# CarbonMatrixLab/AbX

Hardware: AMD Instinct MI355X
Metric: diffusion-steps/sec (100 samples, ~350-res complex) (higher is better)
Workload: dtype f32; 1 GPU; L352: L=352 (Lab 228 + antigen 124), 100 samples of one complex over 1 GPU(s), 1 step = ScoreNetwork (3 passes) + get_prev + reverse, seeded random weights, ESM off; L=352, samples_total=100, chunk=auto, parallelism=sample-shard x1, no collective in the step

## Files before the change

abx_amd/_lib.py:

```python
import ctypes as C
import os

_HERE = os.path.dirname(os.path.abspath(__file__))
LIB_PATH = os.environ.get('ABX_HIP_LIB') or os.path.join(_HERE, 'csrc', 'libabx_hip.so')

c_f = C.c_void_p
LL = C.c_longlong
I = C.c_int
F = C.c_float


class AbxGemm(C.Structure):
    _fields_ = [
        ('A', c_f), ('sAb', LL), ('sAm', LL), ('sAk', LL),
        ('B', c_f), ('sBb', LL), ('sBk', LL), ('sBn', LL),
        ('C', c_f), ('sCb', LL), ('sCm', LL),
        ('M', I), ('N', I), ('K', I), ('batch', I),
        ('c_transposed', I),
        ('ln_stats', c_f), ('sSb', LL),
        ('ln_csum', c_f),
        ('ln_eps', F),
        ('a_relu', I),
        ('bias', c_f),
        ('alpha', F),
# ... 94 lines not shown
class AbxLinearPack(C.Structure):
    _fields_ = [('Wt', c_f), ('csum', c_f), ('bias', c_f), ('planes', C.c_void_p), ('b_exp', I), ('K', I), ('N', I)]


class AbxLinearSrc(C.Structure):
    _fields_ = [('W', c_f), ('b', c_f), ('rows', I), ('glu', I)]


class AbxTriMulPack(C.Structure):
    _fields_ = [('glu', AbxLinearPack), ('out', AbxLinearPack), ('gate', AbxLinearPack)]


class AbxTriAttnPack(C.Structure):
    _fields_ = [('qkv', AbxLinearPack), ('gate', AbxLinearPack), ('pair', AbxLinearPack), ('out', AbxLinearPack)]


class AbxScoreArgs(C.Structure):
    _fields_ = [
        ('init_q', c_f), ('init_t', c_f), ('delta_q', c_f), ('cur_t', c_f), ('fixed_mask', c_f),
        ('t', c_f), ('t_is_f32', I),
        ('score_norms', c_f), ('num_sigma', I), ('num_omega', I), ('discrete_sigma', c_f), ('discrete_omega', c_f),
        ('exp_max_sigma', F), ('exp_min_sigma', F),
        ('min_b', F), ('bdiff', F),
        ('coord_scale', F),
        ('position_scale', F),
        ('rot_score', c_f), ('trans_score', c_f), ('rigids', c_f),
        ('B', I), ('L', I),
    ]


class AbxReverseArgs(C.Structure):
    _fields_ = [
        ('rigid_in', c_f), ('rigid_is_f64', I),
        ('seq_in', c_f),
        ('rot_score', c_f), ('trans_score', c_f), ('ts_is_f32', I), ('logits', c_f),
        ('diffuse_mask', c_f), ('t', c_f), ('dt', F),
        ('z_rot', c_f), ('z_trans', c_f), ('jumps', c_f),
        ('u_jumps', c_f),
        ('dt_dev', c_f),
        ('seed', C.c_ulonglong), ('sample_ids', c_f), ('step', I),
        ('step_dev', c_f),
        ('exp_max_sigma', F), ('exp_min_sigma', F), ('min_b', F), ('bdiff', F), ('coord_scale', F), ('rate_const', F),
        ('noise_scale', F), ('center', I),
        ('rigid_out', c_f), ('seq_out', c_f), ('rates_out', c_f), ('jumps_out', c_f),
        ('B', I), ('L', I),
    ]


class AbxGuidanceArgs(C.Structure):
    _fields_ = [
        ('atom14', c_f), ('atom_mask', c_f), ('aatype', c_f), ('chain_id', c_f),
        ('residx', c_f),
        ('radius', c_f), ('frame_trans', c_f),
        ('overlap_tolerance', F), ('between_chain_factor', F), ('bond_tolerance_factor', F), ('w_clash', F), ('w_bond', F), ('w_angle', F),
        ('energy', c_f), ('grad_atom', c_f), ('grad_trans', c_f), ('grad_rot', c_f),
        ('B', I), ('L', I),
    ]


_S = c_f

_PROTOS = {
    'abx_version': (I, []),
    'abx_last_error_string': (C.c_char_p, []),
    'abx_init': (I, [I]),
    'abx_gemm': (I, [C.POINTER(AbxGemm), _S]),
    'abx_gemm_side': (I, [C.POINTER(AbxGemm), C.POINTER(AbxGemm), _S]),
    'abx_gemm_check_modes': (I, [C.POINTER(AbxGemm)]),
    'abx_gemm_planes_ok': (I, [LL]),
    'abx_split_weights_f16': (I, [c_f, LL, LL, I, I, I, C.c_void_p, _S]),
    'abx_ipa_tail': (I, [C.POINTER(AbxIpaTail), _S]),
    'abx_heads_tail': (I, [C.POINTER(AbxHeadsTail), _S]),
    'abx_gemm3_occupancy': (I, [I]),
    'abx_row_stats': (I, [c_f, LL, LL, LL, I, I, I, F, c_f, _S]),
    'abx_layernorm': (I, [c_f, LL, LL, I, c_f, c_f, F, c_f, LL, c_f, LL, _S]),
    'abx_tri_attn_fwd': (I, [C.POINTER(AbxTriAttn), _S]),
    'abx_seq_attn_fwd': (I, [c_f, c_f, c_f, c_f, c_f, I, I, I, I, F, _S]),
    'abx_ipa_pack': (I, [c_f, c_f, c_f, c_f, c_f, c_f, I, I, F, _S]),
    'abx_ipa_attn': (I, [c_f, c_f, c_f, c_f, c_f, c_f, c_f, c_f, c_f, c_f, c_f, I, I, _S]),
    'abx_debug_poison_lds': (I, [C.c_uint, _S]),
    'abx_ipa_weights': (I, [c_f, c_f, c_f, c_f, c_f, c_f, c_f, c_f, c_f, c_f, I, I, _S]),
    'abx_ipa_pair': (I, [c_f, c_f, c_f, I, I, _S]),
    'abx_ipa_attn_workspace_bytes': (C.c_longlong, [I, I]),
    'abx_ipa_qpack_bytes': (C.c_longlong, [I, I]),
    'abx_timestep_embedding': (I, [c_f, c_f, I, I, c_f, _S]),
    'abx_assemble_seq': (I, [c_f, LL, c_f, c_f, I, c_f, c_f, c_f, c_f, c_f, I, I, I, I, _S]),
    'abx_assemble_pair': (I, [c_f, LL, c_f, c_f, c_f, c_f, c_f, c_f, c_f, c_f, I, I, I, I, _S]),
    'abx_opm_features': (I, [c_f, c_f, LL, c_f, I, I, I, _S]),
    'abx_opm_out_fwd': (I, [c_f, LL, c_f, c_f, c_f, I, I, c_f, I, _S]),
    'abx_assemble_pair_bias': (I, [c_f, LL, c_f, c_f, c_f, c_f, c_f, c_f, c_f, C.c_void_p, I, c_f, c_f, F, c_f, I, I, c_f, I, _S]),
    'abx_pair_mask': (I, [c_f, c_f, I, I, I, _S]),
    'abx_transpose_last2': (I, [c_f, c_f, I, I, I, I, _S]),
    'abx_pair_embed_features': (I, [c_f, c_f, c_f, c_f, c_f, c_f, c_f, c_f, c_f, c_f, c_f, c_f, I, I, _S]),
    'abx_relpos_block': (I, [c_f, c_f, c_f, I, I, I, I, I, _S]),
    'abx_gather_rows': (I, [c_f, c_f, c_f, c_f, LL, LL, I, _S]),
    'abx_frames_init': (I, [c_f, I, c_f, c_f, c_f, c_f, c_f, c_f, I, F, _S]),
    'abx_rigid_update': (I, [c_f, c_f, c_f, c_f, c_f, c_f, c_f, c_f, I, F, _S]),
    'abx_scores': (I, [C.POINTER(AbxScoreArgs), _S]),
    'abx_torsion_finalize': (I, [c_f, c_f, c_f, c_f, I, _S]),
    'abx_seq_head_atoms': (I, [c_f, c_f, c_f, c_f, c_f, c_f, c_f, c_f, c_f, c_f, c_f, c_f, I, _S]),
    'abx_prev_pos': (I, [c_f, c_f, I, c_f, I, I, _S]),
    'abx_plddt': (I, [c_f, c_f, I, I, _S]),
    'abx_igso3_tables': (I, [c_f, c_f, I, I, I, c_f, c_f, c_f, _S]),
    'abx_reverse_step': (I, [C.POINTER(AbxReverseArgs), _S]),
    'abx_clash_grad_workspace_bytes': (LL, [I, I]),
    'abx_clash_grad': (I, [C.POINTER(AbxGuidanceArgs), c_f, _S]),
    'abx_pack_linear_bytes': (LL, [I, I]),
    'abx_pack_linear': (I, [C.POINTER(AbxLinearSrc), I, I, c_f, c_f, I, c_f, C.POINTER(AbxLinearPack), _S]),
    'abx_transition_workspace_bytes': (LL, [LL, I, I]),
    'abx_transition_fwd': (I, [C.POINTER(AbxLinearPack), C.POINTER(AbxLinearPack), c_f, LL, I, c_f, c_f, I, _S]),
    'abx_tri_mul_workspace_bytes': (LL, [I, I]),
    'abx_tri_mul_workspace_init': (I, [c_f, I, I, _S]),
    'abx_tri_mul_fwd': (I, [C.POINTER(AbxTriMulPack), c_f, c_f, c_f, I, I, I, c_f, c_f, I, _S]),
    'abx_tri_attn_block_workspace_bytes': (LL, [I, I]),
    'abx_tri_attn_block_fwd': (I, [C.POINTER(AbxTriAttnPack), c_f, c_f, I, I, I, I, c_f, c_f, I, _S]),
}

EXPORTED = tuple(_PROTOS)
_lib = None


class AbxHipError(RuntimeError):
    pass


def library_path():
    return LIB_PATH


def load():
    global _lib
    if _lib is not None:
        return _lib
    if not os.path.exists(LIB_PATH):
        raise AbxHipError(f'{LIB_PATH} not found: build it with `make -C abx_amd/csrc` (no CPU fallback exists)')
    lib = C.CDLL(LIB_PATH)
    for name, (res, args) in _PROTOS.items():
        fn = getattr(lib, name)
        fn.restype = res
        fn.argtypes = args
    if lib.abx_version() != 1:
        raise AbxHipError('libabx_hip ABI version mismatch')
    _lib = lib
    return lib


def check(rc, what):
    if rc != 0:
        msg = load().abx_last_error_string()
        raise AbxHipError(f'{what} failed (rc={rc}): {msg.decode() if msg else ""}')
```

abx_amd/csrc/ipa.hip:

```cpp
#include "common.h"
#include "abx_hip.h"

namespace {

constexpr int H = 12, SQK = 16, SV = 16, PQK = 4, PV = 8, CZ = 128;
constexpr int QREC = SQK + 3 * PQK;
constexpr int VREC = SV + 3 * PV;
constexpr int NPROJ = H * SQK + H * (SQK + SV) + 3 * H * PQK + 3 * H * (PQK + PV);
constexpr int OFF_KV = H * SQK;
constexpr int OFF_QP = OFF_KV + H * (SQK + SV);
constexpr int OFF_KVP = OFF_QP + 3 * H * PQK;
constexpr int NFEAT = H * SV + 3 * H * PV + H * PV + H * CZ;

constexpr int IPA_THREADS = 512;
constexpr int IQ = 12;
constexpr int HG = 4, NHG = H / HG;

__global__ __launch_bounds__(256) void ipa_pack_kernel(const float* __restrict__ proj, const float* __restrict__ rots,
                                                       const float* __restrict__ trans, float* __restrict__ qpack,
                                                       float* __restrict__ kpack, float* __restrict__ vpack, int B, int L,
                                                       float w_s) {
    const int NIB = (L + IQ - 1) / IQ, LQ = NIB * IQ;
    const long long idx = (long long)blockIdx.x * 256 + threadIdx.x;
    if (idx >= (long long)B * LQ * H) return;
// ... 267 lines not shown
        const long long row = (long long)b * L + i0 + iq;
        const float* R = rots + row * 9;
        const float* t = trans + row * 3;
        const float* g = opt + (iq * HG + hl) * VREC + SV + pt * 3;
        float loc[3];
#pragma unroll
        for (int r = 0; r < 3; ++r) {
            const float it = -(R[0 * 3 + r] * t[0] + R[1 * 3 + r] * t[1] + R[2 * 3 + r] * t[2]);
            loc[r] = it + (R[0 * 3 + r] * g[0] + R[1 * 3 + r] * g[1] + R[2 * 3 + r] * g[2]);
        }
        float* fo = feat + row * NFEAT;
#pragma unroll
        for (int r = 0; r < 3; ++r) fo[H * SV + r * (H * PV) + n] = loc[r];
        fo[H * SV + 3 * H * PV + n] = sqrtf(loc[0] * loc[0] + loc[1] * loc[1] + loc[2] * loc[2] + 1e-8f);
    }
    ISTAMP(7)
}

constexpr int PAIR_WAVES = 4;
#ifndef ABX_PAIR_UZ
#define ABX_PAIR_UZ 8
#endif
constexpr int UZ = ABX_PAIR_UZ;

__global__ __launch_bounds__(PAIR_WAVES * 64) void ipa_pair_kernel(const float* __restrict__ attn, const float* __restrict__ z,
                                                                   float* __restrict__ feat, long long rows, int L) {
    typedef float f32x2 __attribute__((ext_vector_type(2)));
    __shared__ __attribute__((aligned(16))) float wl[PAIR_WAVES][UZ * H];
    const int lane = threadIdx.x & 63, wave = threadIdx.x >> 6;
    const long long row = (long long)blockIdx.x * PAIR_WAVES + wave;
    if (row >= rows) return;
    const float* __restrict__ wr = attn + row * L * H;
    const float* __restrict__ zr = z + row * L * CZ + lane * 2;
    float* ws = wl[wave];
    const int nw = L * HG;
    f32x2 acc[H];
#pragma unroll
    for (int h = 0; h < H; ++h) acc[h] = (f32x2){0.f, 0.f};
    f32x2 za[UZ], zb[UZ];
    float wa[NHG], wb[NHG];
    auto request = [&](int j0, f32x2 (&zd)[UZ], float (&wd)[NHG]) {
#pragma unroll
        for (int u = 0; u < UZ; ++u) zd[u] = *reinterpret_cast<const f32x2*>(zr + (long long)min(j0 + u, L - 1) * CZ);
#pragma unroll
        for (int q = 0; q < NHG; ++q) wd[q] = wr[(long long)q * nw + min(j0 * HG + (lane & (UZ * HG - 1)), nw - 1)];
    };
    auto sum_step = [&](int j0, const f32x2 (&zd)[UZ], const float (&wd)[NHG]) {
#pragma unroll
        for (int q = 0; q < NHG; ++q) ws[q * (UZ * HG) + (lane & (UZ * HG - 1))] = wd[q];
        __builtin_amdgcn_fence(__ATOMIC_RELEASE, "wavefront");
        __builtin_amdgcn_wave_barrier();
        __builtin_amdgcn_fence(__ATOMIC_ACQUIRE, "wavefront");
#pragma unroll
        for (int u = 0; u < UZ; ++u) {
            if (j0 + u < L) {
                f32x4 w4[H / 4];
#pragma unroll
                for (int q = 0; q < NHG; ++q) w4[q] = *reinterpret_cast<const f32x4*>(ws + q * (UZ * HG) + u * HG);
#pragma unroll
                for (int h = 0; h < H; ++h) {
                    const float wh = w4[h >> 2][h & 3];
                    acc[h][0] = fmaf(wh, zd[u][0], acc[h][0]);
                    acc[h][1] = fmaf(wh, zd[u][1], acc[h][1]);
                }
            }
        }
        __builtin_amdgcn_fence(__ATOMIC_RELEASE, "wavefront");
        __builtin_amdgcn_wave_barrier();
    };
    request(0, za, wa);
    for (int j0 = 0; j0 < L; j0 += 2 * UZ) {
        if (j0 + UZ < L) request(j0 + UZ, zb, wb);
        sum_step(j0, za, wa);
        if (j0 + UZ < L) {
            if (j0 + 2 * UZ < L) request(j0 + 2 * UZ, za, wa);
            sum_step(j0 + UZ, zb, wb);
        }
    }
    float* fo = feat + row * NFEAT + (H * SV + 4 * H * PV) + lane * 2;
#pragma unroll
    for (int h = 0; h < H; ++h) *reinterpret_cast<f32x2*>(fo + h * CZ) = acc[h];
}

}

extern "C" int abx_ipa_pack(const float* proj, const float* rots, const float* trans, float* qpack, float* kpack,
                            float* vpack, int B, int L, float scalar_weight, hipStream_t st) {
    ABX_REQUIRE(proj && rots && trans && qpack && kpack && vpack && B > 0 && L > 0, "abx_ipa_pack: bad args");
    const long long n = (long long)B * ((L + IQ - 1) / IQ) * IQ * H;
    hipLaunchKernelGGL(ipa_pack_kernel, dim3((unsigned)((n + 255) / 256)), dim3(256), 0, st, proj, rots, trans, qpack, kpack,
                       vpack, B, L, scalar_weight);
    return abx_check_launch("abx_ipa_pack");
}

extern "C" long long abx_ipa_qpack_bytes(int B, int L) {
    return (long long)B * ((L + IQ - 1) / IQ) * IQ * H * QREC * sizeof(float);
}

extern "C" long long abx_ipa_attn_workspace_bytes(int B, int L) {
    return (long long)B * L * L * H * sizeof(float);
}

extern "C" int abx_ipa_weights(const float* qpack, const float* kpack, const float* vpack, const float* bias2d, const float* mask,
                               const float* rots, const float* trans, const float* point_weights, float* attn_ws, float* feat, int B,
                               int L, hipStream_t st) {
    ABX_REQUIRE(qpack && kpack && vpack && bias2d && mask && rots && trans && point_weights && attn_ws && feat, "abx_ipa_weights: null");
    ABX_REQUIRE(B > 0 && L > 0 && B <= 65535 && (long long)B * L < (1ll << 31), "abx_ipa_weights: bad sizes");
    const size_t lds = (ipa_logits_floats(L) + IQ * HG * VREC) * sizeof(float);
    ABX_REQUIRE(lds <= 160 * 1024, "abx_ipa_weights: L too large for LDS-resident logits");
    if (int rc = abx_ensure_dynamic_lds(reinterpret_cast<const void*>(ipa_weights_kernel), 160 * 1024, "abx_ipa_weights")) return rc;
    const long long per_b = (long long)((L + IQ - 1) / IQ) * NHG;
    const long long nwg = 8 * ((B / 8) * per_b + ((B % 8) * per_b + 7) / 8);
    ABX_REQUIRE(nwg < (1LL << 31), "abx_ipa_weights: grid too large");
    hipLaunchKernelGGL(ipa_weights_kernel, dim3((unsigned)nwg), dim3(IPA_THREADS), lds, st, qpack, kpack, vpack, bias2d, mask,
                       rots, trans, point_weights, attn_ws, feat, B, L);
    return abx_check_launch("abx_ipa_weights");
}

#ifdef IPA_STAMP
extern "C" int abx_ipa_stamps(unsigned long long* out) {
    return (int)hipMemcpyFromSymbol(out, HIP_SYMBOL(ipa_stamp_buf), sizeof(unsigned long long) * 1024 * 8);
}
#endif

extern "C" int abx_ipa_pair(const float* attn_ws, const float* z, float* feat, int B, int L, hipStream_t st) {
    ABX_REQUIRE(attn_ws && z && feat && B > 0 && L > 0 && (long long)B * L < (1ll << 31), "abx_ipa_pair: bad args");
    const long long rows = (long long)B * L;
    hipLaunchKernelGGL(ipa_pair_kernel, dim3((unsigned)((rows + PAIR_WAVES - 1) / PAIR_WAVES)), dim3(PAIR_WAVES * 64), 0, st, attn_ws, z,
                       feat, rows, L);
    return abx_check_launch("abx_ipa_pair");
}

extern "C" int abx_ipa_attn(const float* qpack, const float* kpack, const float* vpack, const float* bias2d, const float* z,
                            const float* mask, const float* rots, const float* trans, const float* point_weights, float* attn_ws,
                            float* feat, int B, int L, hipStream_t st) {
    ABX_REQUIRE(z != nullptr, "abx_ipa_attn: null");
    const int rc = abx_ipa_weights(qpack, kpack, vpack, bias2d, mask, rots, trans, point_weights, attn_ws, feat, B, L, st);
    if (rc) return rc;
    return abx_ipa_pair(attn_ws, z, feat, B, L, st);
}
```

abx_amd/ops.py:

```python
import ctypes as C
import math

import torch

from abx_amd import _lib
from abx_amd._lib import (AbxGemm, AbxTriAttn, AbxIpaTail, AbxHeadsTail, AbxScoreArgs, AbxReverseArgs, AbxGuidanceArgs, AbxLinearPack, AbxLinearSrc,
                           AbxTriMulPack, AbxTriAttnPack, check)


def _stream():
    return C.c_void_p(torch.cuda.current_stream().cuda_stream)


def _p(t):
    if t is None:
        return None
    assert t.is_cuda, 'libabx_hip works on device memory only'
    return t.data_ptr()


def _f32(t):
    assert t.dtype == torch.float32, t.dtype
    return t

# ... 567 lines not shown


def ipa_tail(feat, s, w_final, ln1, w_t0, w_t2, w_t4, ln2, eps=1e-5, affine=None, rigid=None, partial=None):
    M, K1 = feat.shape
    assert s.shape == (M, 256) and feat.stride(1) == 1 and s.stride(1) == 1 and K1 % 16 == 0
    a = AbxIpaTail()
    a.feat, a.s_feat, a.s, a.s_s, a.M, a.K1, a.C = _p(_f32(feat)), feat.stride(0), _p(_f32(s)), s.stride(0), M, K1, 256
    if partial is not None:
        assert partial.dim() == 3 and partial.shape[1:] == (M, 256) and partial.is_contiguous()
        a.partial, a.n_partial, a.s_partial = _p(_f32(partial)), partial.shape[0], M * 256
    for tag, (w3, bias), K in (('final', w_final, K1), ('t0', w_t0, 256), ('t2', w_t2, 256), ('t4', w_t4, 256)):
        _weight_planes(w3, 256, K, what='ipa_tail ' + tag)
        assert w3.shape[0] * 16 == K and bias.numel() == 256
        setattr(a, 'W_' + tag, _p(w3)); setattr(a, 'e_' + tag, w3.w_exp); setattr(a, 'b_' + tag, _p(_f32(bias)))
    a.ln1_w, a.ln1_b, a.ln2_w, a.ln2_b = _p(_f32(ln1[0])), _p(_f32(ln1[1])), _p(_f32(ln2[0])), _p(_f32(ln2[1]))
    a.ln_eps = float(eps)
    if affine is not None:
        wa, ba = affine
        fixed, init_q, init_t, cur_q, cur_t, cur_R, delta_q, pscale = rigid
        assert wa.shape == (256, 6) and wa.is_contiguous() and ba.numel() == 6 and fixed.dtype == torch.int32 and fixed.numel() == M
        a.W_aff, a.b_aff, a.fixed = _p(_f32(wa)), _p(_f32(ba)), _p(fixed)
        a.init_q, a.init_t, a.cur_q, a.cur_t, a.cur_R, a.delta_q = [_p(_f32(t)) for t in (init_q, init_t, cur_q, cur_t, cur_R, delta_q)]
        a.pscale = float(pscale)
    if RANGE_CHECK:
        a.range_flag, a.range_tag = range_ptr(s.device), RANGE_TAGS['ipa_tail']
    check(_lib.load().abx_ipa_tail(C.byref(a), _stream()), 'abx_ipa_tail')
    return s


def pad_planes_128(wt, bias):
    K, n = wt.shape
    w = torch.zeros(K, 128, device=wt.device, dtype=torch.float32)
    w[:, :n] = wt
    b = torch.zeros(128, device=wt.device, dtype=torch.float32)
    if bias is not None:
        b[:n] = bias
    return split_weights(w), b


def heads_tail(s, s0, torsion, seq_head, plddt_head, un, logits, pl=None, eps=1e-5):
    M = s.shape[0]
    assert s.shape == (M, 256) and s0.shape == (M, 256) and s.stride(1) == 1 and s0.stride(1) == 1
    assert un.shape == (M, 14) and un.is_contiguous() and logits.shape == (M, 20) and logits.is_contiguous()
    a = AbxHeadsTail()
    a.s, a.s_s, a.s0, a.s_s0, a.M = _p(_f32(s)), s.stride(0), _p(_f32(s0)), s0.stride(0), M
    keep = []

    def put(tag, wb, K):
        w3, bias = wb
        _weight_planes(w3, 128, K, what='heads_tail ' + tag)
        assert w3.shape[0] * 16 == K and bias.numel() == 128
        setattr(a, 'W_' + tag, _p(w3)); setattr(a, 'e_' + tag, w3.w_exp); setattr(a, 'b_' + tag, _p(_f32(bias)))
        keep.append((w3, bias))
    for tag, wb, K in zip(('act', 'init', 'r0', 'r1', 'r2', 'r3', 'proj'), torsion, (256, 256, 128, 128, 128, 128, 128)):
        put(tag, wb, K)
    (g_s, b_s), *lin_s = seq_head
    a.lns_w, a.lns_b = _p(_f32(g_s)), _p(_f32(b_s))
    for tag, wb, K in zip(('s1', 's3', 's5'), lin_s, (256, 128, 128)):
        put(tag, wb, K)
    a.un, a.logits = _p(_f32(un)), _p(_f32(logits))
    if pl is not None:
        assert pl.shape == (M, 50) and pl.is_contiguous()
        (g_p, b_p), *lin_p = plddt_head
        a.lnp_w, a.lnp_b = _p(_f32(g_p)), _p(_f32(b_p))
        for tag, wb, K in zip(('p1', 'p3', 'p5'), lin_p, (256, 128, 128)):
            put(tag, wb, K)
        a.pl = _p(_f32(pl))
    a.ln_eps = float(eps)
    if RANGE_CHECK:
        a.range_flag, a.range_tag = range_ptr(s.device), RANGE_TAGS['heads_tail']
    check(_lib.load().abx_heads_tail(C.byref(a), _stream()), 'abx_heads_tail')


def ipa_qpack_numel(B, L):
    return _lib.load().abx_ipa_qpack_bytes(B, L) // 4


def ipa_pack(proj, rots, trans, qpack, kpack, vpack, B, L, w_s):
    assert qpack.numel() >= ipa_qpack_numel(B, L)
    check(_lib.load().abx_ipa_pack(_p(proj), _p(rots), _p(trans), _p(qpack), _p(kpack), _p(vpack), B, L, float(w_s), _stream()),
          'abx_ipa_pack')


def ipa_attn(qpack, kpack, vpack, bias2d, z, mask, rots, trans, pw, feat, B, L, attn_ws=None):
    if attn_ws is None:
        attn_ws = torch.empty(_lib.load().abx_ipa_attn_workspace_bytes(B, L) // 4, device=feat.device, dtype=torch.float32)
    assert attn_ws.numel() >= B * L * L * 12 and attn_ws.is_contiguous()
    check(_lib.load().abx_ipa_attn(_p(qpack), _p(kpack), _p(vpack), _p(bias2d), _p(z), _p(mask), _p(rots), _p(trans), _p(pw),
                                   _p(attn_ws), _p(feat), B, L, _stream()), 'abx_ipa_attn')


_FREQS = {}


def timestep_embedding(t64, dim, out):
    import math
    assert t64.dtype == torch.float64
    key = (dim, str(t64.device))
    if key not in _FREQS:
        half = dim // 2
        _FREQS[key] = torch.exp(torch.arange(half, dtype=torch.float32) * -(math.log(10000) / (half - 1))).to(t64.device)
    check(_lib.load().abx_timestep_embedding(_p(t64), _p(_FREQS[key]), t64.shape[0], dim, _p(out), _stream()),
          'abx_timestep_embedding')
    return out


def assemble_seq(seq_static, aa_table, seq_t, Lab, temb, prev_seq, gamma, beta, out, B, L, C_, E):
    ss_b = 0 if seq_static.shape[0] == 1 else seq_static.stride(0)
    assert seq_t.dtype == torch.int64 and seq_t.is_contiguous()
    check(_lib.load().abx_assemble_seq(_p(seq_static), ss_b, _p(aa_table), _p(seq_t), Lab, _p(temb), _p(prev_seq), _p(gamma),
                                       _p(beta), _p(out), B, L, C_, E, _stream()), 'abx_assemble_seq')
    return out


def assemble_pair(pair_static, temb, prev_pair, gamma, beta, prev_pos, pos_table, out, B, L, C_, E, stats_out=None):
    ps_b = 0 if pair_static.shape[0] == 1 else pair_static.stride(0)
    if prev_pos is not None:
        assert prev_pos.dtype == torch.int64 and prev_pos.is_contiguous()
    check(_lib.load().abx_assemble_pair(_p(pair_static), ps_b, _p(temb), _p(prev_pair), _p(gamma), _p(beta), _p(prev_pos),
                                        _p(pos_table), _p(out), _p(stats_out), B, L, C_, E, _stream()), 'abx_assemble_pair')
    return out


def assemble_pair_bias(pair_static, temb, prev_pair, gamma, beta, prev_pos, pos_table, out, w3, csum, bias, biasT, B, L, range_class='gemm'):
    ps_b = 0 if pair_static.shape[0] == 1 else pair_static.stride(0)
    assert out.is_contiguous() and out.shape[-1] == 192 and pair_static.shape[-1] == 128 and temb.shape[-1] == 32
    assert tuple(w3.shape) == (12, 2, 32, 16) and biasT.is_contiguous() and biasT.numel() == B * 32 * L * L and csum.numel() == 32
    if prev_pos is not None:
        assert prev_pos.dtype == torch.int64 and prev_pos.is_contiguous()
    flag, tag = (range_ptr(out.device), RANGE_TAGS[range_class]) if RANGE_CHECK else (None, 0)
    check(_lib.load().abx_assemble_pair_bias(_p(pair_static), ps_b, _p(temb), _p(prev_pair), _p(gamma), _p(beta), _p(prev_pos), _p(pos_table), _p(out),
                                             _p(w3), w3.w_exp, _p(_f32(csum)), _p(bias), 1e-5, _p(biasT), B, L, flag, tag, _stream()),
          'abx_assemble_pair_bias')
    return out


def opm_features(lr, feat, B, L, C_=64):
    es = lr.element_size()
    check(_lib.load().abx_opm_features(lr.data_ptr(), lr.data_ptr() + C_ * es, lr.stride(0), _p(feat), B, L, C_, _stream()),
          'abx_opm_features')
    return feat


def opm_out(lr, Wt, bias, z, B, L, range_class='gemm'):
    assert lr.shape[1] == 128 and tuple(Wt.shape) == (128, 192) and Wt.is_contiguous() and z.is_contiguous() and z.shape[-1] == 192
    flag, tag = (range_ptr(z.device), RANGE_TAGS[range_class]) if RANGE_CHECK else (None, 0)
    check(_lib.load().abx_opm_out_fwd(_p(_f32(lr)), lr.stride(0), _p(_f32(Wt)), _p(bias), _p(_f32(z)), B, L, flag, tag, _stream()), 'abx_opm_out_fwd')
    return z


def pair_mask(mask_f, out, B, L, Lp=None):
    check(_lib.load().abx_pair_mask(_p(mask_f), _p(out), B, L, L if Lp is None else Lp, _stream()), 'abx_pair_mask')
    return out


def gather_rows(table, idx, out, rowscale=None):
    idx = idx.reshape(-1)
    assert idx.dtype == torch.int64 and idx.is_contiguous() and table.is_contiguous()
    n, C_ = idx.numel(), table.shape[1]
    check(_lib.load().abx_gather_rows(_p(table), _p(idx), _p(rowscale), _p(out), out.stride(0), n, C_, _stream()), 'abx_gather_rows')
    return out


def relpos_block(residx, table, out, B, L, Lab, max_rel):
    assert residx.dtype == torch.int32 and residx.is_contiguous()
    check(_lib.load().abx_relpos_block(_p(residx), _p(table), _p(out), B, L, Lab, table.shape[1], max_rel, _stream()),
# ... 119 lines not shown
```

include/abx_hip.h:

```cpp
#ifndef ABX_HIP_H
#define ABX_HIP_H

#include <stdint.h>
#ifdef __HIPCC__
#include <hip/hip_runtime.h>
#else
typedef struct ihipStream_t* hipStream_t;
#endif

#ifdef __cplusplus
extern "C" {
#endif

#define ABX_HIP_ABI_VERSION 1

int abx_version(void);
const char* abx_last_error_string(void);
int abx_init(int device);
int abx_debug_poison_lds(unsigned pattern, hipStream_t stream);

typedef struct AbxGemm {
    const float* A; long long sAb, sAm, sAk;
    const float* B; long long sBb, sBk, sBn;
    float* C;       long long sCb, sCm;
// ... 42 lines not shown
typedef struct AbxIpaTail {
    const float* feat; long long s_feat;
    float* s; long long s_s;
    int M, K1, C;
    const unsigned short* W_final; int e_final; const float* b_final;
    const float* ln1_w; const float* ln1_b;
    const unsigned short* W_t0; int e_t0; const float* b_t0;
    const unsigned short* W_t2; int e_t2; const float* b_t2;
    const unsigned short* W_t4; int e_t4; const float* b_t4;
    const float* ln2_w; const float* ln2_b;
    float ln_eps;
    const float* W_aff; const float* b_aff;
    const int* fixed; const float* init_q; const float* init_t;
    float* cur_q; float* cur_t; float* cur_R; float* delta_q; float pscale;
    int* range_flag; int range_tag;
    const float* partial; int n_partial; long long s_partial;
} AbxIpaTail;
int abx_ipa_tail(const AbxIpaTail* desc, hipStream_t stream);
typedef struct AbxHeadsTail {
    const float* s; long long s_s;
    const float* s0; long long s_s0;
    int M;
    const unsigned short* W_act; int e_act; const float* b_act;
    const unsigned short* W_init; int e_init; const float* b_init;
    const unsigned short* W_r0; int e_r0; const float* b_r0;
    const unsigned short* W_r1; int e_r1; const float* b_r1;
    const unsigned short* W_r2; int e_r2; const float* b_r2;
    const unsigned short* W_r3; int e_r3; const float* b_r3;
    const unsigned short* W_proj; int e_proj; const float* b_proj;
    float* un;
    const float* lns_w; const float* lns_b;
    const unsigned short* W_s1; int e_s1; const float* b_s1;
    const unsigned short* W_s3; int e_s3; const float* b_s3;
    const unsigned short* W_s5; int e_s5; const float* b_s5;
    float* logits;
    const float* lnp_w; const float* lnp_b;
    const unsigned short* W_p1; int e_p1; const float* b_p1;
    const unsigned short* W_p3; int e_p3; const float* b_p3;
    const unsigned short* W_p5; int e_p5; const float* b_p5;
    float* pl;
    float ln_eps;
    int* range_flag; int range_tag;
} AbxHeadsTail;
int abx_heads_tail(const AbxHeadsTail* desc, hipStream_t stream);
int abx_gemm3_occupancy(int which);

int abx_row_stats(const float* x, long long s_b, long long s_row, long long s_k, int batch, int rows, int K, float eps,
                  float* stats, hipStream_t stream);
int abx_layernorm(const float* x, long long s_row, long long rows, int K, const float* gamma, const float* beta, float eps,
                  float* out, long long s_out, const float* res, long long s_res, hipStream_t stream);

typedef struct AbxTriAttn {
    const float* q; const float* k; const float* v; const float* gate;
    long long sb, ss, sl;
    const float* bias; long long bias_sb, bias_sh, bias_sq, bias_sk;
    const float* keymask; long long km_sb;
    float* out; long long ob, os, ol;
    int B, S, L, H, D;
    float scale;
    int exact;
    unsigned long long* clock_probe;
    int* range_flag; int range_tag;
    int tune;
    int bias_log2;
    int kv_planes;
    int q_parts, row_groups;
} AbxTriAttn;
#define ABX_TRI_BIAS_LOG2 (1.4426950408889634f * 128.0f)
int abx_tri_attn_fwd(const AbxTriAttn* desc, hipStream_t stream);

int abx_seq_attn_fwd(const float* qkv, const float* bias, const float* keymask, const float* gate, float* out, int B, int L,
                     int H, int D, float scale, hipStream_t stream);

int abx_ipa_pack(const float* proj, const float* rots, const float* trans, float* qpack, float* kpack, float* vpack,
                 int B, int L, float scalar_weight, hipStream_t stream);
int abx_ipa_attn(const float* qpack, const float* kpack, const float* vpack, const float* bias2d, const float* z,
                 const float* mask, const float* rots, const float* trans, const float* point_weights ,
                 float* attn_ws, float* feat, int B, int L, hipStream_t stream);
int abx_ipa_weights(const float* qpack, const float* kpack, const float* vpack, const float* bias2d, const float* mask,
                    const float* rots, const float* trans, const float* point_weights, float* attn_ws, float* feat, int B, int L,
                    hipStream_t stream);
int abx_ipa_pair(const float* attn_ws, const float* z, float* feat, int B, int L, hipStream_t stream);
long long abx_ipa_attn_workspace_bytes(int B, int L);
long long abx_ipa_qpack_bytes(int B, int L);

int abx_timestep_embedding(const double* t, const float* freqs, int B, int dim, float* out, hipStream_t stream);
int abx_assemble_seq(const float* seq_static, long long ss_b, const float* aa_table, const long long* seq_t, int Lab,
                     const float* temb, const float* prev_seq, const float* gamma, const float* beta, float* out, int B,
                     int L, int C, int E, hipStream_t stream);
int abx_assemble_pair(const float* pair_static, long long ps_b, const float* temb, const float* prev_pair,
                      const float* gamma, const float* beta, const long long* prev_pos, const float* pos_table, float* out,
                      float* stats_out, int B, int L, int C, int E, hipStream_t stream);
int abx_assemble_pair_bias(const float* pair_static, long long ps_b, const float* temb, const float* prev_pair, const float* gamma,
                           const float* beta, const long long* prev_pos, const float* pos_table, float* out, const unsigned short* w_planes,
                           int w_exp, const float* csum, const float* bias, float ln_eps, float* biasT, int B, int L, int* range_flag,
                           int range_tag, hipStream_t stream);
int abx_opm_features(const float* left, const float* right, long long ld, float* feat, int B, int L, int C,
                     hipStream_t stream);
int abx_opm_out_fwd(const float* lr, long long ld, const float* Wt, const float* bias, float* z, int B, int L, int* range_flag, int range_tag,
                    hipStream_t stream);
int abx_transpose_last2(const float* in, float* out, int nmat, int L, int Lp, int transpose, hipStream_t stream);
int abx_pair_mask(const float* mask, float* out, int B, int L, int Lp, hipStream_t stream);

int abx_pair_embed_features(const long long* aa, const int* chain_id, const int* residx, const float* atom14,
                            const unsigned char* atom14_exists, const float* aa_pair_embed, const float* relpos_embed,
                            const float* distcoef, const float* dgram_embed, const float* sq_breaks ,
                            float* feat512, float* dist196, int B, int L, hipStream_t stream);
int abx_relpos_block(const int* residx, const float* table, float* out, int B, int L, int Lab, int C, int max_rel,
                     hipStream_t stream);
int abx_gather_rows(const float* table, const long long* idx, const float* rowscale, float* out, long long s_out, long long n,
                    int C, hipStream_t stream);

int abx_frames_init(const void* rigids_t, int is_f64, float* init_q, float* init_t, float* cur_q, float* cur_t, float* cur_R,
                    float* delta_q, int n, float position_scale, hipStream_t stream);
int abx_rigid_update(const float* upd6, const int* fixed_mask, const float* init_q, const float* init_t, float* cur_q,
                     float* cur_t, float* cur_R, float* delta_q, int n, float position_scale, hipStream_t stream);
typedef struct AbxScoreArgs {
    const float* init_q; const float* init_t; const float* delta_q; const float* cur_t; const int* fixed_mask;
    const double* t; int t_is_f32;
    const float* score_norms; int num_sigma, num_omega; const float* discrete_sigma; const float* discrete_omega;
    float exp_max_sigma, exp_min_sigma;
    float min_b, bdiff;
    float coord_scale;
    float position_scale;
    float* rot_score; void* trans_score; float* rigids;
    int B, L;
} AbxScoreArgs;
int abx_scores(const AbxScoreArgs* a, hipStream_t stream);
int abx_torsion_finalize(const float* unnorm, const float* gt_sincos, const int* fixed_mask, float* angles, int n,
                         hipStream_t stream);
int abx_seq_head_atoms(const float* logits, const int* fixed_mask, const long long* seq_t, const float* rigids,
                       const float* angles, const long long* atom37_to_atom14, const float* default_frames,
                       const int* group_idx, const float* lit_pos, long long* seq_0, float* atom14, float* atom37, int n,
                       hipStream_t stream);
int abx_prev_pos(const float* atom37, const float* sq_breaks, int num_breaks, long long* prev_pos, int B, int L,
                 hipStream_t stream);
int abx_plddt(const float* logits, float* out, int n, int bins, hipStream_t stream);

int abx_igso3_tables(const float* sigma, const float* omega, int num_sigma, int num_omega, int L_terms, float* pdf, float* cdf,
                     float* score_norms, hipStream_t stream);
typedef struct AbxReverseArgs {
    const void* rigid_in; int rigid_is_f64;
    const long long* seq_in;
    const float* rot_score; const void* trans_score; int ts_is_f32; const float* logits;
    const int* diffuse_mask; const double* t; float dt;
    const float* z_rot; const float* z_trans; const float* jumps;
    const float* u_jumps;
    const float* dt_dev;
    unsigned long long seed; const long long* sample_ids; int step;
    const int* step_dev;
    float exp_max_sigma, exp_min_sigma, min_b, bdiff, coord_scale, rate_const;
    float noise_scale; int center;
    double* rigid_out; long long* seq_out; float* rates_out; float* jumps_out;
    int B, L;
} AbxReverseArgs;
int abx_reverse_step(const AbxReverseArgs* a, hipStream_t stream);

typedef struct AbxGuidanceArgs {
    const float* atom14; const unsigned char* atom_mask; const long long* aatype; const int* chain_id;
    const int* residx;
    const float* radius; const float* frame_trans;
    float overlap_tolerance, between_chain_factor, bond_tolerance_factor, w_clash, w_bond, w_angle;
    float* energy;
    float* grad_atom; float* grad_trans; float* grad_rot;
    int B, L;
} AbxGuidanceArgs;
// ... 37 lines not shown
```

Measured before the change: 167.2 sample-steps/s.

## Fuse IPA attention weights and pair aggregation into one LDS-resident kernel

Adds an ipa_fused_kernel that handles four query rows per workgroup entirely in LDS. It computes scalar and point logits, adds the pair bias and mask, runs the softmax, then aggregates the z pair features, the value vectors and the point outputs, including the inverse-frame transform. The goal is to stop writing and re-reading the B*L*L*H attention-weight workspace in global memory and to save one kernel launch. In exchange, each workgroup re-reads the full key and value arrays for only four query rows, and LDS use near 80 KB may limit occupancy. The old two-kernel path stays as a fallback when the logits do not fit in LDS.

```diff
diff --git a/abx_amd/_lib.py b/abx_amd/_lib.py
--- a/abx_amd/_lib.py
+++ b/abx_amd/_lib.py
@@ -200,6 +200,7 @@
     'abx_ipa_weights': (I, [c_f, c_f, c_f, c_f, c_f, c_f, c_f, c_f, c_f, c_f, I, I, _S]),
     'abx_ipa_pair': (I, [c_f, c_f, c_f, I, I, _S]),
     'abx_ipa_attn_workspace_bytes': (C.c_longlong, [I, I]),
+    'abx_ipa_attn_fused': (I, [I]),
     'abx_ipa_qpack_bytes': (C.c_longlong, [I, I]),
     'abx_timestep_embedding': (I, [c_f, c_f, I, I, c_f, _S]),
     'abx_assemble_seq': (I, [c_f, LL, c_f, c_f, I, c_f, c_f, c_f, c_f, c_f, I, I, I, I, _S]),
diff --git a/abx_amd/csrc/ipa.hip b/abx_amd/csrc/ipa.hip
--- a/abx_amd/csrc/ipa.hip
+++ b/abx_amd/csrc/ipa.hip
@@ -373,6 +373,271 @@
     for (int h = 0; h < H; ++h) *reinterpret_cast<f32x2*>(fo + h * CZ) = acc[h];
 }
 
+constexpr int FQ = 4;
+constexpr int FRED_I = FQ * 4 + 4;
+constexpr int FRED_G = (H * VREC / 4) * FRED_I + 4;
+constexpr int FUZ = 16;
+constexpr size_t IPA_FUSED_LDS_MAX = 80 * 1024;
+__host__ __device__ inline size_t ipa_fused_logits_floats(int L) {
+    const size_t lgf = (size_t)FQ * H * ipa_row_stride(L), redf = (size_t)6 * FRED_G;
+    return lgf > redf ? lgf : redf;
+}
+inline size_t ipa_fused_lds_bytes(int L) { return (ipa_fused_logits_floats(L) + FQ * H * VREC) * sizeof(float); }
+
+__global__ __launch_bounds__(IPA_THREADS, 4) void ipa_fused_kernel(const float* __restrict__ qpack, const float* __restrict__ kpack,
+                                                                   const float* __restrict__ vpack, const float* __restrict__ bias2d,
+                                                                   const float* __restrict__ z, const float* __restrict__ mask,
+                                                                   const float* __restrict__ rots, const float* __restrict__ trans,
+                                                                   const float* __restrict__ pw, float* __restrict__ feat, int B, int L) {
+    extern __shared__ __attribute__((aligned(16))) float smem[];
+    const int LR = ipa_row_stride(L);
+    float* lg = smem;
+    float* opt = smem + ipa_fused_logits_floats(L);
+    const int tid = threadIdx.x, lane = tid & 63, wave = tid >> 6;
+    const int NIB = (L + IQ - 1) / IQ, per_b = (L + FQ - 1) / FQ;
+    const int xcd = blockIdx.x & 7, slot = blockIdx.x >> 3;
+    const int full_slots = (B / 8) * per_b;
+    int b, wb;
+    if (slot < full_slots) {
+        b = (slot / per_b) * 8 + xcd;
+        wb = slot % per_b;
+    } else {
+        const int t = (slot - full_slots) * 8 + xcd;
+        if (t >= (B % 8) * per_b) return;
+        b = (B / 8) * 8 + t / per_b;
+        wb = t % per_b;
+    }
+    const int i0 = wb * FQ;
+    const int niq = min(FQ, L - i0);
+
+    {
+        typedef float f32x2 __attribute__((ext_vector_type(2)));
+        const float* __restrict__ qb = qpack + ((long long)b * NIB + i0 / IQ) * H * (IQ / 2) * (QREC * 2) + (i0 % IQ) / 2 * (QREC * 2);
+        const int wpk = (L + 63) >> 6;
+        for (int task = wave; task < H * wpk; task += IPA_THREADS / 64) {
+            const int h = __builtin_amdgcn_readfirstlane(task / wpk);
+            const int j = (task - h * wpk) * 64 + lane;
+            const float* kr = kpack + (((long long)b * H + h) * L + min(j, L - 1)) * QREC;
+            f32x4 kq[QREC / 4];
+#pragma unroll
+            for (int c4 = 0; c4 < QREC / 4; ++c4) kq[c4] = *reinterpret_cast<const f32x4*>(kr + c4 * 4);
+            const float pwh = pw[h];
+            const f32x2* __restrict__ qh = reinterpret_cast<const f32x2*>(qb + (long long)h * (IQ / 2) * (QREC * 2));
+#pragma unroll
+            for (int ip = 0; ip < FQ / 2; ++ip) {
+                f32x2 sacc = {0.f, 0.f}, d2 = {0.f, 0.f};
+#pragma unroll
+                for (int c = 0; c < SQK; ++c) {
+                    const float kc = kq[c >> 2][c & 3];
+                    sacc = __builtin_elementwise_fma(qh[ip * QREC + c], (f32x2){kc, kc}, sacc);
+                }
+#pragma unroll
+                for (int c = SQK; c < QREC; ++c) {
+                    const float kc = kq[c >> 2][c & 3];
+                    const f32x2 d = qh[ip * QREC + c] - (f32x2){kc, kc};
+                    d2 = __builtin_elementwise_fma(d, d, d2);
+                }
+                if (j < L) {
+                    lg[(size_t)((2 * ip) * H + h) * LR + j] = sacc[0] + pwh * d2[0];
+                    lg[(size_t)((2 * ip + 1) * H + h) * LR + j] = sacc[1] + pwh * d2[1];
+                }
+            }
+        }
+    }
+    __syncthreads();
+    for (int idx = tid; idx < niq * L; idx += IPA_THREADS) {
+        const int iq = idx / L, j = idx - iq * L;
+        const long long row = (long long)b * L + i0 + iq;
+        const f32x4* bz = reinterpret_cast<const f32x4*>(bias2d + (row * L + j) * H);
+        const bool masked = mask[row] * mask[(long long)b * L + j] == 0.f;
+        float* r = lg + (size_t)iq * H * LR + j;
+#pragma unroll
+        for (int g = 0; g < NHG; ++g) {
+            const f32x4 bg = bz[g];
+#pragma unroll
+            for (int c = 0; c < HG; ++c) r[(size_t)(g * HG + c) * LR] = masked ? ABX_NEG_MAX : r[(size_t)(g * HG + c) * LR] + bg[c];
+        }
+    }
+    __syncthreads();
+    {
+        constexpr int SH = H / 2;
+        const int iq = wave >> 1;
+        if (iq < niq) {
+            float* r = lg + (size_t)(iq * H + (wave & 1) * SH) * LR;
+            float mx[SH], sm[SH], inv[SH];
+#pragma unroll
+            for (int c = 0; c < SH; ++c) { mx[c] = -INFINITY; sm[c] = 0.f; }
+            for (int j = lane; j < L; j += 64)
+#pragma unroll
+                for (int c = 0; c < SH; ++c) mx[c] = fmaxf(mx[c], r[(size_t)c * LR + j]);
+#pragma unroll
+            for (int c = 0; c < SH; ++c) mx[c] = wave_max(mx[c]);
+            for (int j = lane; j < L; j += 64)
+#pragma unroll
+                for (int c = 0; c < SH; ++c) {
+                    const float e = expf(r[(size_t)c * LR + j] - mx[c]);
+                    r[(size_t)c * LR + j] = e;
+                    sm[c] += e;
+                }
+#pragma unroll
+            for (int c = 0; c < SH; ++c) inv[c] = 1.0f / wave_sum(sm[c]);
+            for (int j = lane; j < L; j += 64)
+#pragma unroll
+                for (int c = 0; c < SH; ++c) r[(size_t)c * LR + j] *= inv[c];
+        }
+    }
+    __syncthreads();
+    {
+        const int iq = wave >> 1;
+        if (iq < niq) {
+            const long long row = (long long)b * L + i0 + iq;
+            const float* __restrict__ zr = z + row * L * CZ + (wave & 1) * 64 + lane;
+            const float* wrow = lg + (size_t)iq * H * LR;
+            float acc[H];
+#pragma unroll
+            for (int h = 0; h < H; ++h) acc[h] = 0.f;
+            float za[FUZ], zb[FUZ];
+            auto request = [&](int j0, float (&zd)[FUZ]) {
+#pragma unroll
+                for (int u = 0; u < FUZ; ++u) zd[u] = zr[(long long)min(j0 + u, L - 1) * CZ];
+            };
+            auto sum_step = [&](int j0, const float (&zd)[FUZ]) {
+#pragma unroll
+                for (int u4 = 0; u4 < FUZ; u4 += 4) {
+                    f32x4 w4[H];
+#pragma unroll
+                    for (int h = 0; h < H; ++h) w4[h] = *reinterpret_cast<const f32x4*>(wrow + (size_t)h * LR + j0 + u4);
+#pragma unroll
+                    for (int u = 0; u < 4; ++u) {
+                        if (j0 + u4 + u < L) {
+#pragma unroll
+                            for (int h = 0; h < H; ++h) acc[h] = fmaf(w4[h][u], zd[u4 + u], acc[h]);
+                        }
+                    }
+                }
+            };
+            request(0, za);
+            for (int j0 = 0; j0 < L; j0 += 2 * FUZ) {
+                if (j0 + FUZ < L) request(j0 + FUZ, zb);
+                sum_step(j0, za);
+                if (j0 + FUZ < L) {
+                    if (j0 + 2 * FUZ < L) request(j0 + 2 * FUZ, za);
+                    sum_step(j0 + FUZ, zb);
+                }
+            }
+            float* fo = feat + row * NFEAT + (H * SV + 4 * H * PV) + (wave & 1) * 64 + lane;
+#pragma unroll
+            for (int h = 0; h < H; ++h) fo[h * CZ] = acc[h];
+        }
+    }
+    constexpr int NJG = 12, IPW = 5, UB = 4;
+    const int il = lane % IPW, jg = lane / IPW;
+    const int item0 = wave * IPW + il;
+    const int hl1 = item0 / (VREC / 4), c41 = item0 % (VREC / 4);
+    f32x4 acc[NHG][FQ];
+#pragma unroll
+    for (int p = 0; p < NHG; ++p) {
+#pragma unroll
+        for (int iq = 0; iq < FQ; ++iq) acc[p][iq] = (f32x4){0.f, 0.f, 0.f, 0.f};
+        if (jg < NJG) {
+            const int h = p * HG + hl1;
+            const float* vb = vpack + ((long long)b * H + h) * L * VREC + c41 * 4;
+            const float* wr = lg + (size_t)h * LR;
+            f32x4 vnext[UB];
+            auto load_round = [&](int jb) {
+#pragma unroll
+                for (int u = 0; u < UB; ++u) vnext[u] = *reinterpret_cast<const f32x4*>(vb + (long long)min(jb + u * NJG, L - 1) * VREC);
+            };
+            load_round(jg);
+            for (int jb = jg; jb < L; jb += NJG * UB) {
+                f32x4 vv[UB];
+#pragma unroll
+                for (int u = 0; u < UB; ++u) vv[u] = vnext[u];
+                if (jb + NJG * UB < L) load_round(jb + NJG * UB);
+#pragma unroll
+                for (int u = 0; u < UB; ++u) {
+                    const int j = jb + u * NJG;
+                    if (j < L) {
+#pragma unroll
+                        for (int iq = 0; iq < FQ; ++iq) {
+                            const float w = wr[(size_t)iq * H * LR + j];
+#pragma unroll
+                            for (int c = 0; c < 4; ++c) acc[p][iq][c] = fmaf(w, vv[u][c], acc[p][iq][c]);
+                        }
+                    }
+                }
+            }
+        }
+    }
+    {
+        float* red = lg;
+        auto slot_of = [&](int g, int p) { return red + (size_t)g * FRED_G + (size_t)(p * HG * (VREC / 4) + item0) * FRED_I; };
+        auto put = [&](int g) {
+#pragma unroll
+            for (int p = 0; p < NHG; ++p)
+#pragma unroll
+                for (int iq = 0; iq < FQ; ++iq) *reinterpret_cast<f32x4*>(slot_of(g, p) + iq * 4) = acc[p][iq];
+        };
+        auto add = [&](int g) {
+#pragma unroll
+            for (int p = 0; p < NHG; ++p)
+#pragma unroll
+                for (int iq = 0; iq < FQ; ++iq) {
+                    const f32x4 o4 = *reinterpret_cast<const f32x4*>(slot_of(g, p) + iq * 4);
+#pragma unroll
+                    for (int c = 0; c < 4; ++c) acc[p][iq][c] += o4[c];
+                }
+        };
+        __syncthreads();
+        if (jg >= 6 && jg < NJG) put(jg - 6);
+        __syncthreads();
+        if (jg < 6) add(jg);
+        __syncthreads();
+        if (jg >= 3 && jg < 6) put(jg - 3);
+        __syncthreads();
+        if (jg < 3) add(jg);
+        __syncthreads();
+        if (jg == 1 || jg == 2) put(jg - 1);
+        __syncthreads();
+        if (jg == 0) {
+#pragma unroll
+            for (int p = 0; p < NHG; ++p) {
+                const int h = p * HG + hl1;
+#pragma unroll
+                for (int iq = 0; iq < FQ; ++iq) {
+                    const f32x4 x1 = *reinterpret_cast<const f32x4*>(slot_of(0, p) + iq * 4), x2 = *reinterpret_cast<const f32x4*>(slot_of(1, p) + iq * 4);
+#pragma unroll
+                    for (int c = 0; c < 4; ++c) acc[p][iq][c] = (acc[p][iq][c] + x1[c]) + x2[c];
+                    *reinterpret_cast<f32x4*>(opt + (size_t)(iq * H + h) * VREC + c41 * 4) = acc[p][iq];
+                }
+            }
+        }
+        __syncthreads();
+    }
+    for (int idx = tid; idx < niq * H * SV; idx += IPA_THREADS) {
+        const int iq = idx / (H * SV), r = idx % (H * SV);
+        feat[((long long)b * L + i0 + iq) * NFEAT + r] = opt[(iq * H + r / SV) * VREC + (r % SV)];
+    }
+    for (int idx = tid; idx < niq * H * PV; idx += IPA_THREADS) {
+        const int iq = idx / (H * PV), n = idx % (H * PV);
+        const int h = n / PV, pt = n % PV;
+        const long long row = (long long)b * L + i0 + iq;
+        const float* R = rots + row * 9;
+        const float* t = trans + row * 3;
+        const float* g = opt + (iq * H + h) * VREC + SV + pt * 3;
+        float loc[3];
+#pragma unroll
+        for (int r = 0; r < 3; ++r) {
+            const float it = -(R[0 * 3 + r] * t[0] + R[1 * 3 + r] * t[1] + R[2 * 3 + r] * t[2]);
+            loc[r] = it + (R[0 * 3 + r] * g[0] + R[1 * 3 + r] * g[1] + R[2 * 3 + r] * g[2]);
+        }
+        float* fo = feat + row * NFEAT;
+#pragma unroll
+        for (int r = 0; r < 3; ++r) fo[H * SV + r * (H * PV) + n] = loc[r];
+        fo[H * SV + 3 * H * PV + n] = sqrtf(loc[0] * loc[0] + loc[1] * loc[1] + loc[2] * loc[2] + 1e-8f);
+    }
+}
+
 }
 
 extern "C" int abx_ipa_pack(const float* proj, const float* rots, const float* trans, float* qpack, float* kpack,
@@ -426,7 +691,21 @@
                             const float* mask, const float* rots, const float* trans, const float* point_weights, float* attn_ws,
                             float* feat, int B, int L, hipStream_t st) {
     ABX_REQUIRE(z != nullptr, "abx_ipa_attn: null");
-    const int rc = abx_ipa_weights(qpack, kpack, vpack, bias2d, mask, rots, trans, point_weights, attn_ws, feat, B, L, st);
-    if (rc) return rc;
-    return abx_ipa_pair(attn_ws, z, feat, B, L, st);
-}
+    if (L > 0 && ipa_fused_lds_bytes(L) > IPA_FUSED_LDS_MAX) {
+        const int rc = abx_ipa_weights(qpack, kpack, vpack, bias2d, mask, rots, trans, point_weights, attn_ws, feat, B, L, st);
+        if (rc) return rc;
+        return abx_ipa_pair(attn_ws, z, feat, B, L, st);
+    }
+    ABX_REQUIRE(qpack && kpack && vpack && bias2d && mask && rots && trans && point_weights && feat, "abx_ipa_attn: null");
+    ABX_REQUIRE(B > 0 && L > 0 && B <= 65535 && (long long)B * L < (1ll << 31), "abx_ipa_attn: bad sizes");
+    const size_t lds = ipa_fused_lds_bytes(L);
+    if (int rc = abx_ensure_dynamic_lds(reinterpret_cast<const void*>(ipa_fused_kernel), (int)IPA_FUSED_LDS_MAX, "abx_ipa_attn")) return rc;
+    const long long per_b = (L + FQ - 1) / FQ;
+    const long long nwg = 8 * ((B / 8) * per_b + ((B % 8) * per_b + 7) / 8);
+    ABX_REQUIRE(nwg < (1LL << 31), "abx_ipa_attn: grid too large");
+    hipLaunchKernelGGL(ipa_fused_kernel, dim3((unsigned)nwg), dim3(IPA_THREADS), lds, st, qpack, kpack, vpack, bias2d, z, mask, rots,
+                       trans, point_weights, feat, B, L);
+    return abx_check_launch("abx_ipa_attn");
+}
+
+extern "C" int abx_ipa_attn_fused(int L) { return L > 0 && ipa_fused_lds_bytes(L) <= IPA_FUSED_LDS_MAX; }
diff --git a/abx_amd/ops.py b/abx_amd/ops.py
--- a/abx_amd/ops.py
+++ b/abx_amd/ops.py
@@ -673,6 +673,10 @@
           'abx_ipa_pack')
 
 
+def ipa_attn_fused(L):
+    return bool(_lib.load().abx_ipa_attn_fused(L))
+
+
 def ipa_attn(qpack, kpack, vpack, bias2d, z, mask, rots, trans, pw, feat, B, L, attn_ws=None):
     if attn_ws is None:
         attn_ws = torch.empty(_lib.load().abx_ipa_attn_workspace_bytes(B, L) // 4, device=feat.device, dtype=torch.float32)
diff --git a/include/abx_hip.h b/include/abx_hip.h
--- a/include/abx_hip.h
+++ b/include/abx_hip.h
@@ -148,6 +148,7 @@
                     hipStream_t stream);
 int abx_ipa_pair(const float* attn_ws, const float* z, float* feat, int B, int L, hipStream_t stream);
 long long abx_ipa_attn_workspace_bytes(int B, int L);
+int abx_ipa_attn_fused(int L);
 long long abx_ipa_qpack_bytes(int B, int L);
 
 int abx_timestep_embedding(const double* t, const float* freqs, int B, int dim, float* out, hipStream_t stream);
```

Result: no change. 167.3 sample-steps/s, median of 4 (+0.0%).
